# borglab/gtsfm

Measured on NVIDIA H100. Metric: image_pairs_per_sec, higher is better.
Workload: dtype f32

## Files before the change

gtsfm_b200/_lib.py:

```python
from __future__ import annotations

import ctypes as C
from pathlib import Path
from typing import Optional

import numpy as np

LIB_PATH = Path(__file__).resolve().parent / "libgtsfm_b200.so"

_lib: Optional[C.CDLL] = None


class B200Error(RuntimeError):
    pass


class LightGlueParams(C.Structure):
    _fields_ = [("depth_confidence", C.c_double), ("width_confidence", C.c_double), ("filter_threshold", C.c_double),
                ("prune_min_kpts", C.c_int), ("fp16_attention", C.c_int)]


class LightGluePair(C.Structure):
    _fields_ = [("kp0", C.c_void_p), ("desc0", C.c_void_p), ("n0", C.c_int), ("kp1", C.c_void_p), ("desc1", C.c_void_p), ("n1", C.c_int),
                ("out_matches", C.c_void_p), ("out_scores", C.c_void_p), ("out_k", C.c_int), ("out_stop_layer", C.c_int),
# ... 131 lines not shown
                ("R_error_deg", C.c_double), ("U_error_deg", C.c_double)]


class ViewGraphParams(C.Structure):
    _fields_ = [("criterion", C.c_int), ("pad_", C.c_int), ("error_threshold_deg", C.c_double)]


VG_MEDIAN, VG_MIN = 0, 1

_vp, _i, _f, _sz = C.c_void_p, C.c_int, C.c_float, C.c_size_t
_ip = C.POINTER(C.c_int)

SIGNATURES = {
    "b2_version": (_i, []),
    "b2_create": (_i, [_i, C.POINTER(_vp)]),
    "b2_destroy": (None, [_vp]),
    "b2_last_error": (C.c_char_p, [_vp]),
    "b2_launch_count": (C.c_uint64, [_vp]),
    "b2_h2d_bytes": (C.c_uint64, [_vp]),
    "b2_set_option": (C.c_int, [_vp, C.c_char_p, C.c_int64]),
    "b2_profile_start": (_i, [_vp, C.c_char_p]),
    "b2_profile_stop": (_i, [_vp, C.POINTER(C.c_double), C.POINTER(C.c_uint64), C.POINTER(C.c_double)]),
    "b2_debug_fetch": (C.c_int64, [_vp, C.c_char_p, _vp, C.c_int64]),
    "b2_debug_linear_host": (_i, [_vp, C.POINTER(LinearLaunch), C.POINTER(LinearProblem), _i]),
    "b2_debug_conv_host": (_i, [_vp, C.POINTER(ConvLayer)]),
    "b2_debug_gemm_segments_host": (_i, [_vp, _vp, _vp, _vp, _i, _i, _i, _i, _vp, _vp, _i, _vp, _vp]),
    "b2_debug_attention_host": (_i, [_vp, _i, _ip, _ip, _i, _f, _i, _vp, _vp, _vp, _vp]),
    "b2_debug_superglue_assign_host": (_i, [_vp, _i, _i, _vp, _i, _i, _f, _i, _f, _vp, _vp, _vp, _vp, _vp, _vp, _vp, _ip, _ip]),
    "b2_debug_lightglue_assign_host": (_i, [_vp, _i, _i, _vp, _i, _i, _vp, _vp, _vp, _vp, _f, _vp, _vp, _vp, _vp, _vp, _vp, _vp, _ip,
                                            _ip]),
    "b2_debug_lightglue_argmax_host": (_i, [_vp, _i, _vp, _i, _i, _vp, _vp, _vp, _vp, _vp, _ip]),
    "b2_debug_lightglue_posenc_host": (_i, [_vp, _i, _vp, _vp, _vp, _vp, _vp, _vp]),
    "b2_debug_lightglue_ln_gelu_host": (_i, [_vp, _i, _vp, _vp, _vp, _vp, _vp, _vp]),
    "b2_debug_lightglue_rowheads_host": (_i, [_vp, _i, _vp, _vp, _vp, _vp, _vp, _vp, _vp, _vp, _vp, _vp]),
    "b2_debug_lightglue_prune_host": (_i, [_vp, _i, _vp, _vp, _vp, _f, _f, _vp, _vp]),
    "b2_debug_lightglue_gather_host": (_i, [_vp, _i, _vp, _vp, _vp, _vp, _vp, _vp, _vp, _vp, _vp, _vp, _vp, _vp, _vp]),
    "b2_debug_lightglue_filter_host": (_i, [_vp, _i, _i, _vp, _vp, _vp, _f, _vp, _vp, _vp, _vp, _ip]),
    "b2_superpoint_set_weights": (_i, [_vp, _vp, _sz]),
    "b2_superpoint_detect_dev": (_i, [_vp, _vp, _i, _i, _i, _sz, _f, _i, _i, _vp, _vp, _i, _ip, C.POINTER(C.c_uint64), _vp]),
    "b2_superpoint_describe_dev": (_i, [_vp, C.c_uint64, _vp, _i, _vp, _vp]),
    "b2_superpoint_extract_dev": (_i, [_vp, _vp, _i, _i, _i, _sz, _f, _i, _i, _i, _vp, _vp, _vp, _ip, _vp]),
    "b2_superpoint_extract_async_dev": (_i, [_vp, _vp, _i, _i, _i, _sz, _f, _i, _i, _i, _vp, _vp, _vp, _vp, _vp]),
    "b2_superpoint_finish_dev": (_i, [_vp, _vp]),
    "b2_superpoint_detect_host": (_i, [_vp, _vp, _i, _i, _i, _f, _i, _i, _vp, _vp, _i, _ip, C.POINTER(C.c_uint64)]),
    "b2_superpoint_describe_host": (_i, [_vp, C.c_uint64, _vp, _i, _vp]),
    "b2_image_resize_dev": (_i, [_vp, _vp, _i, _i, _i, _sz, _vp, _i, _i, _vp]),
    "b2_lightglue_set_weights": (_i, [_vp, _vp, _sz]),
    "b2_lightglue_qkv_rows": (_i, [_vp]),
    "b2_lightglue_match_dev": (_i, [_vp, _vp, _vp, _i, _vp, _vp, _i, C.POINTER(LightGlueParams), _vp, _vp, _ip, _ip, _vp]),
    "b2_lightglue_match_host": (_i, [_vp, _vp, _vp, _i, _vp, _vp, _i, C.POINTER(LightGlueParams), _vp, _vp, _ip, _ip]),
    "b2_lightglue_match_batched_dev": (_i, [_vp, C.POINTER(LightGluePair), _i, C.POINTER(LightGlueParams), _vp]),
    "b2_lightglue_trace_count": (_i, [_vp]),
    "b2_lightglue_trace_get": (_i, [_vp, _i, _vp, _vp, _vp, _vp, _vp, _vp]),
    "b2_lightglue_encoded_bytes": (_sz, [_i]),
    "b2_lightglue_encode_batched_dev": (_i, [_vp, C.POINTER(LightGlueImage), _i, C.POINTER(LightGlueParams), _vp]),
    "b2_superglue_set_weights": (_i, [_vp, _vp, _sz]),
    "b2_superglue_match_dev": (_i, [_vp, _vp, _vp, _vp, _i, _i, _i, _vp, _vp, _vp, _i, _i, _i, _i, _f, _vp, _vp, _ip, _vp]),
    "b2_superglue_match_host": (_i, [_vp, _vp, _vp, _vp, _i, _i, _i, _vp, _vp, _vp, _i, _i, _i, _i, _f, _vp, _vp, _ip]),
    "b2_netvlad_blob_floats": (_sz, []),
    "b2_netvlad_set_weights": (_i, [_vp, _vp, _sz]),
    "b2_netvlad_describe_dev": (_i, [_vp, _vp, _i, _i, _i, _vp, _vp]),
    "b2_netvlad_describe_host": (_i, [_vp, _vp, _i, _i, _i, _vp]),
    "b2_megaloc_blob_floats": (_sz, []),
    "b2_megaloc_set_weights": (_i, [_vp, _vp, _sz]),
    "b2_megaloc_describe_dev": (_i, [_vp, _vp, _i, _i, _i, _vp, _vp]),
    "b2_megaloc_describe_host": (_i, [_vp, _vp, _i, _i, _i, _vp]),
# ... 131 lines not shown
```

gtsfm_b200/csrc/lightglue.cu:

```cuda
#include <stdlib.h>

#include "common.cuh"
#include "linear.cuh"
#include "assign_ps.cuh"

namespace {
constexpr int LG_LAYERS = 9;
constexpr size_t LG_NFLOATS = 11851601;
constexpr int D = 256;

struct SelfW {
  float *wqkv, *bqkv, *wout, *bout, *w0, *b0, *lng, *lnb, *w3, *b3;
};
struct CrossW {
  float *wqv, *bqv, *wout, *bout, *w0, *b0, *lng, *lnb, *w3, *b3;
};
struct AssignW {
  float *wm, *bm, *wf, *bf;
};
struct ConfW {
  float *w, *b;
};
}

constexpr int LG_MAX_PAIRS = 8;
constexpr int LG_MAX_SIDES = 2 * LG_MAX_PAIRS;
static_assert(LG_MAX_SIDES <= GW_MAXP && LG_MAX_SIDES <= AP_MAXP, "batch does not fit one launch");

struct LgSide {
  DevBuf x[2], xs[2], qkv, q, k, v, ctx, msg, h, hs, cs[2], sn[2], ind[2], conf, mat, src, md, rmax, rlog, ls, lsg, amax, aidx;
  int cur = 0;
  int n = 0;
  int cap = 0;
};

struct LgPair {
  bool active = false;
  int n0 = 0, n1 = 0;
  int stop = 0;
  long long* out_matches = nullptr;
  float* out_scores = nullptr;
};

struct LgTraceRec {
  int pair = 0, side = 0, layer = 0, n = 0;
  int heads = 0;
  int unconf = 0, kept = 0, stop = 0;
  std::vector<float> x, conf, mat;
  std::vector<int> ind, keep;
};

struct LightGlueState {
  bool loaded = false;
  int persist_ctas = 132;
  DevBuf wblob, wblob_h, wblob_l, errflag;
  bool use_tc = true;
  float* wr = nullptr;
  SelfW sw[LG_LAYERS];
  CrossW cw[LG_LAYERS];
  AssignW aw[LG_LAYERS];
  ConfW tw[LG_LAYERS - 1];
  float thr[LG_LAYERS];
  LgSide side[LG_MAX_SIDES];
// ... 589 lines not shown
  B2_CUDA(ctx, s->wblob.ensure(total * sizeof(float)));
  B2_CUDA(ctx, cudaMemcpy(s->wblob.p, host.data(), total * sizeof(float), cudaMemcpyHostToDevice));
  float* base = s->wblob.as<float>();
  size_t ti = 0;
  auto next = [&]() { return base + doff[ti++]; };
  s->wr = next();
  for (int i = 0; i < LG_LAYERS; ++i) {
    SelfW& a = s->sw[i];
    a.wqkv = next(), a.bqkv = next(), a.wout = next(), a.bout = next(), a.w0 = next(), a.b0 = next(), a.lng = next(),
    a.lnb = next(), a.w3 = next(), a.b3 = next();
    CrossW& c = s->cw[i];
    c.wqv = next(), c.bqv = next(), next(), next();
    c.wout = next(), c.bout = next(), c.w0 = next(), c.b0 = next(), c.lng = next(), c.lnb = next(), c.w3 = next(), c.b3 = next();
  }
  for (int i = 0; i < LG_LAYERS; ++i) {
    AssignW& a = s->aw[i];
    a.wm = next(), a.bm = next(), a.wf = next(), a.bf = next();
  }
  for (int i = 0; i < LG_LAYERS - 1; ++i) s->tw[i].w = next(), s->tw[i].b = next();
  for (int i = 0; i < LG_LAYERS; ++i) {
    double t = 0.8 + 0.1 * exp(-4.0 * i / LG_LAYERS);
    t = t < 0 ? 0 : (t > 1 ? 1 : t);
    s->thr[i] = (float)t;
  }
  B2_CUDA(ctx, s->wblob_h.ensure(total * sizeof(__half)));
  B2_CUDA(ctx, s->wblob_l.ensure(total * sizeof(__half)));
  B2_CUDA(ctx, s->errflag.ensure(16));
  B2_CUDA(ctx, cudaMemset(s->errflag.p, 0, 16));
  B2_LAUNCH(ctx, k_split_f32, (unsigned)((total + 255) / 256), 256, 0, (cudaStream_t)0, s->wblob.as<float>(), total,
            s->wblob_h.as<__half>(), s->wblob_l.as<__half>());
  B2_CHECK_LAUNCH(ctx);
  B2_CUDA(ctx, cudaDeviceSynchronize());
  B2_CUDA(ctx, cudaFuncSetAttribute(k_gemm_ws, cudaFuncAttributeMaxDynamicSharedMemorySize, (int)GW_SMEM));
  B2_CUDA(ctx, cudaFuncSetAttribute(k_flash_ps<false>, cudaFuncAttributeMaxDynamicSharedMemorySize, (int)AS_SMEM));
  B2_CUDA(ctx, cudaFuncSetAttribute(k_flash_ps<true>, cudaFuncAttributeMaxDynamicSharedMemorySize, (int)AS_SMEM));
  s->use_tc = !b2_force_simt(ctx);
  B2_CUDA(ctx, cudaFuncSetAttribute(k_flash_attn, cudaFuncAttributeMaxDynamicSharedMemorySize, (int)FA_SMEM));
  B2_CUDA(ctx, s->hread.ensure(8 * LG_MAX_PAIRS * sizeof(int)));
  B2_CUDA(ctx, s->counters.ensure(8 * LG_MAX_PAIRS * sizeof(int)));
  B2_CUDA(ctx, cudaMemset(s->counters.p, 0, 8 * LG_MAX_PAIRS * sizeof(int)));
  s->loaded = true;
  return B2_OK;
}

static inline TcWeights lg_tw(LightGlueState* s) {
  TcWeights t{s->wblob.as<float>(), s->wblob_h.as<__half>(), s->wblob_l.as<__half>(), s->errflag.as<int>(), s->use_tc};
  t.attn_part = &s->attn_part, t.attn_ml = &s->attn_ml, t.attn_cnt = &s->attn_cnt, t.sm_count = s->persist_ctas;
  return t;
}

static int lg_side_alloc(b2_context* ctx, LgSide& sd, int n, bool use_tc) {
  const size_t N = (size_t)(n > 0 ? n : 1);
  for (int i = 0; i < 2; ++i) {
    B2_CUDA(ctx, sd.x[i].ensure(N * 256 * 4));
    B2_CUDA(ctx, sd.xs[i].ensure(N * 256 * 4));
    B2_CUDA(ctx, sd.cs[i].ensure(N * 32 * 4));
    B2_CUDA(ctx, sd.sn[i].ensure(N * 32 * 4));
    B2_CUDA(ctx, sd.ind[i].ensure(N * 4));
  }
  if (!use_tc) B2_CUDA(ctx, sd.qkv.ensure(N * 768 * 4));
  B2_CUDA(ctx, sd.q.ensure(N * 256 * 4));
  B2_CUDA(ctx, sd.k.ensure(N * 256 * 4));
  B2_CUDA(ctx, sd.v.ensure(N * 256 * 4));
  B2_CUDA(ctx, sd.ctx.ensure(N * 256 * 4));
  B2_CUDA(ctx, sd.msg.ensure(N * 256 * 4));
  B2_CUDA(ctx, sd.h.ensure(N * 512 * 4));
  B2_CUDA(ctx, sd.hs.ensure(N * 512 * 4));
  B2_CUDA(ctx, sd.md.ensure(N * 256 * 4));
  DevBuf* small[] = {&sd.conf, &sd.mat, &sd.src, &sd.rmax, &sd.rlog, &sd.ls, &sd.lsg, &sd.amax, &sd.aidx};
  for (DevBuf* b : small) B2_CUDA(ctx, b->ensure(N * 4));
  sd.cur = 0;
  sd.n = n;
  sd.cap = n;
  return B2_OK;
}

struct LgActive {
  int side[LG_MAX_SIDES];
  int n = 0;
};
static LgActive lg_active_sides(const LightGlueState* s, int np) {
  LgActive a;
  for (int p = 0; p < np; ++p)
    if (s->pair[p].active) a.side[a.n++] = 2 * p, a.side[a.n++] = 2 * p + 1;
  return a;
}
static int lg_max_n(const LightGlueState* s, const LgActive& act) {
  int mx = 0;
  for (int i = 0; i < act.n; ++i) mx = s->side[act.side[i]].n > mx ? s->side[act.side[i]].n : mx;
  return mx;
}

static int lg_out_and_ffn(b2_context* ctx, cudaStream_t st, LightGlueState* s, const LgActive& act, const char* blk, const float* wout,
                          const float* bout, const float* w0, const float* b0, const float* lng, const float* lnb, const float* w3,
                          const float* b3) {
  int rc;
  const TcWeights tw = lg_tw(s);
  LinArgs o[LG_MAX_SIDES], f0[LG_MAX_SIDES], f3[LG_MAX_SIDES];
  for (int i = 0; i < act.n; ++i) {
    LgSide& sd = s->side[act.side[i]];
    const size_t e = (size_t)sd.cap * 256;
    float* x = sd.x[sd.cur].as<float>();
    LinArgs& a = o[i];
    a.a1f = sd.ctx.as<float>(), a.a1p = planes_of(sd.ctx, e), a.lda1 = 256, a.K1 = 256, a.w = wout, a.ldb = 256, a.bias = bout;
    a.cf = sd.msg.as<float>(), a.ldc = 256, a.cp = planes_of(sd.msg, e), a.ldch = 256, a.M = sd.n, a.N = 256;
    LinArgs& f = f0[i];
    f.a1f = x, f.a1p = planes_of(sd.xs[sd.cur], e), f.lda1 = 256, f.K1 = 256;
    f.a2f = sd.msg.as<float>(), f.a2p = planes_of(sd.msg, e), f.lda2 = 256, f.K2 = 256;
    f.w = w0, f.ldb = 512, f.bias = b0, f.cf = sd.h.as<float>(), f.ldc = 512, f.tc_want_f32 = true, f.M = sd.n, f.N = 512;
    LinArgs& c = f3[i];
    c.a1f = sd.h.as<float>(), c.a1p = planes_of(sd.hs, (size_t)sd.cap * 512), c.lda1 = 512, c.K1 = 512, c.w = w3, c.ldb = 512, c.bias = b3;
    c.resid = x, c.ldr = 256;
    c.cf = x, c.ldc = 256, c.tc_want_f32 = true, c.cp = planes_of(sd.xs[sd.cur], e), c.ldch = 256, c.M = sd.n, c.N = 256;
  }
  const std::string site(blk);
  if ((rc = run_linear(ctx, st, tw, o, act.n, (site + "_out").c_str()))) return rc;
  if ((rc = run_linear(ctx, st, tw, f0, act.n, (site + "_ffn0").c_str()))) return rc;
  {
    JobList<LnJob> lj{};
    for (int i = 0; i < act.n; ++i) {
      LgSide& sd = s->side[act.side[i]];
      const Pl hs = planes_of(sd.hs, (size_t)sd.cap * 512);
      lj.j[i] = {sd.h.as<float>(), sd.n, s->use_tc ? hs.hi : (__half*)nullptr, s->use_tc ? hs.lo : (__half*)nullptr};
    }
    const int mx = lg_max_n(s, act);
    if (mx > 0) {
      B2_LAUNCH(ctx, k_lg_ln_gelu, dim3(cdiv(mx, 8), act.n), 256, 0, st, lj, lng, lnb);
      B2_CHECK_LAUNCH(ctx);
    }
  }
  return run_linear(ctx, st, tw, f3, act.n, (site + "_ffn3").c_str());
}

static int lg_self_layer(b2_context* ctx, cudaStream_t st, LightGlueState* s, const LgActive& act, int layer, bool fp16_attn) {
  const SelfW& w = s->sw[layer];
  const TcWeights tw = lg_tw(s);
  int rc;
  LinArgs q[LG_MAX_SIDES];
  for (int i = 0; i < act.n; ++i) {
    LgSide& sd = s->side[act.side[i]];
    const size_t e = (size_t)sd.cap * 256;
    LinArgs& a = q[i];
    a.a1f = sd.x[sd.cur].as<float>(), a.a1p = planes_of(sd.xs[sd.cur], e), a.lda1 = 256, a.K1 = 256;
    a.w = w.wqkv, a.ldb = 256, a.bias = w.bqkv, a.M = sd.n, a.N = 768;
    if (s->use_tc) {
      a.seg_n = 256, a.seg_p[0] = planes_of(sd.q, e), a.seg_p[1] = planes_of(sd.k, e), a.seg_p[2] = planes_of(sd.v, e);
      a.rot_mask = 3, a.cs = sd.cs[sd.cur].as<float>(), a.sn = sd.sn[sd.cur].as<float>();
      a.head_major = 1, a.lo_unscaled = 1;
    } else {
      a.cf = sd.qkv.as<float>(), a.ldc = 768;
    }
  }
  if ((rc = run_linear(ctx, st, tw, q, act.n, "lg_self_qkv"))) return rc;
  const int mx = lg_max_n(s, act);
  if (!s->use_tc && mx > 0) {
    JobList<RotJob> rj{};
// ... 593 lines not shown
    const int pb = cdiv(mx * 32, 1024);
    B2_LAUNCH(ctx, k_lg_posenc, dim3(pb < 16 ? pb : 16, np), 1024, 0, d.st, pj, dwr);
    B2_CHECK_LAUNCH(ctx);
  }
  return d.finish("b2_debug_lightglue_posenc_host");
}

extern "C" int b2_debug_lightglue_ln_gelu_host(b2_context* ctx, int np, const int* n, const float* g, const float* b, float* h,
                                               uint16_t* hi, uint16_t* lo) {
  int mx, rc;
  if (!ctx || !g || !b || !h || !hi != !lo || lg_dbg_sizes(n, np, &mx)) return B2_ERR_ARG;
  std::lock_guard<std::mutex> lk(ctx->mu);
  cudaSetDevice(ctx->device);
  LgDbg d{ctx, ctx->stream};
  JobList<LnJob> lj{};
  float *dg, *db;
  if ((rc = d.put(g, 512, false, &dg)) || (rc = d.put(b, 512, false, &db))) return rc;
  for (int i = 0, o = 0; i < np; o += n[i++]) {
    LnJob& j = lj.j[i];
    const size_t e = 512 * (size_t)o, ne = 512 * (size_t)n[i];
    j.n = n[i];
    uint16_t *dh = nullptr, *dl = nullptr;
    if ((rc = d.put(h + e, ne, true, &j.h)) || (hi && ((rc = d.put(hi + e, ne, true, &dh)) || (rc = d.put(lo + e, ne, true, &dl)))))
      return rc;
    j.hi = reinterpret_cast<__half*>(dh), j.lo = reinterpret_cast<__half*>(dl);
  }
  if (mx > 0) {
    B2_LAUNCH(ctx, k_lg_ln_gelu, dim3(cdiv(mx, 8), np), 256, 0, d.st, lj, dg, db);
    B2_CHECK_LAUNCH(ctx);
  }
  return d.finish("b2_debug_lightglue_ln_gelu_host");
}

extern "C" int b2_debug_lightglue_rowheads_host(b2_context* ctx, int np, const int* n, const int* mode, const float* x, const float* w1,
                                                const float* b1, const float* w2, const float* b2, float* o1, float* o2, float* zraw) {
  int mx, rc;
  if (!ctx || !mode || !x || !o1 || !o2 || !zraw || !w1 != !b1 || !w2 != !b2 || lg_dbg_sizes(n, np, &mx)) return B2_ERR_ARG;
  std::lock_guard<std::mutex> lk(ctx->mu);
  cudaSetDevice(ctx->device);
  LgDbg d{ctx, ctx->stream};
  JobList<HeadJob> hj{};
  float *dw1, *db1, *dw2, *db2;
  if ((rc = d.put(w1, 256, false, &dw1)) || (rc = d.put(b1, 1, false, &db1)) || (rc = d.put(w2, 256, false, &dw2)) ||
      (rc = d.put(b2, 1, false, &db2)))
    return rc;
  for (int i = 0, o = 0; i < np; o += n[i++]) {
    HeadJob& j = hj.j[i];
    float *dx, *d1, *d2, *dz;
    if ((rc = d.put(x + 256 * (size_t)o, 256 * (size_t)n[i], false, &dx)) || (rc = d.put(o1 + o, (size_t)n[i], true, &d1)) ||
        (rc = d.put(o2 + o, (size_t)n[i], true, &d2)) || (rc = d.put(zraw + o, (size_t)n[i], true, &dz)))
      return rc;
    const bool h2 = (mode[i] & 1) && dw2;
    j = {dx, n[i], h2 ? dw2 : nullptr, h2 ? db2 : nullptr, d1, (mode[i] & 2) ? d2 : nullptr, (mode[i] & 4) ? dz : nullptr};
  }
  if (mx > 0) {
    B2_LAUNCH(ctx, k_lg_rowheads, dim3(cdiv(mx, 8), np), 256, 0, d.st, hj, dw1, db1);
    B2_CHECK_LAUNCH(ctx);
  }
  return d.finish("b2_debug_lightglue_rowheads_host");
}

extern "C" int b2_debug_lightglue_prune_host(b2_context* ctx, int np, const int* n, const float* conf, const float* mat, float thr,
                                             float keep_thr, int* src, int* counters) {
  int mx, rc;
  if (!ctx || !conf || !mat || !src || !counters || lg_dbg_sizes(n, np, &mx)) return B2_ERR_ARG;
  std::lock_guard<std::mutex> lk(ctx->mu);
// ... 108 lines not shown
```

gtsfm_b200/csrc/linear.cuh:

```cuda
#pragma once
#include "attn_ps.cuh"
#include "common.cuh"
#include "gemm.cuh"
#include "gemm_ws.cuh"

struct TcWeights {
  const float* f;
  const __half* h;
  const __half* l;
  int* err;
  bool use_tc;
  DevBuf* attn_part = nullptr;
  DevBuf* attn_ml = nullptr;
  DevBuf* attn_cnt = nullptr;
  int sm_count = 132;
};

struct Pl {
  __half* hi;
  __half* lo;
};
static inline Pl planes_of(const DevBuf& b, size_t elems) { return {b.as<__half>(), b.as<__half>() + elems}; }

struct LinArgs {
  const float* a1f = nullptr;
  Pl a1p{nullptr, nullptr};
  int lda1 = 0, K1 = 0;
  const float* a2f = nullptr;
  Pl a2p{nullptr, nullptr};
  int lda2 = 0, K2 = 0;
  const float* w = nullptr;
  const float* bf = nullptr;
  Pl bp{nullptr, nullptr};
  int ldb = 0;
  const float* bias = nullptr;
  float scale = 1.f;
  const float* resid = nullptr;
  int ldr = 0;
  float* cf = nullptr;
  int ldc = 0;
  Pl cp{nullptr, nullptr};
  int ldch = 0;
  int head_major = 0;
  bool tc_want_f32 = false;
  int relu = 0;
  int gelu = 0;
  int lo_unscaled = 0;
  int M = 0, N = 0;
  int seg_n = 0;
  float* seg_f[GW_SEGS] = {};
  Pl seg_p[GW_SEGS] = {};
  int rot_mask = 0;
  const float *cs = nullptr, *sn = nullptr;
};

static int run_linear(b2_context* ctx, cudaStream_t st, const TcWeights& tw, const LinArgs* a, int np, const char* site = nullptr) {
  if (np <= 0) return B2_OK;
  if (np > GW_MAXP) return b2_fail(ctx, B2_ERR_ARG, "run_linear: too many problems in one launch");
  const LinArgs& a0 = a[0];
  const int nseg = a0.seg_n > 0 ? a0.N / a0.seg_n : 1;
  if (a0.seg_n > 0 && (a0.seg_n % GW_N || a0.N != nseg * a0.seg_n || nseg > GW_SEGS || !a0.head_major || a0.resid || a0.tc_want_f32 ||
                       (a0.rot_mask && (!a0.cs || !a0.sn))))
    return b2_fail(ctx, B2_ERR_ARG, "run_linear: column segments need N = seg_n x (<= 3), seg_n % 128 == 0, head-major planes, "
                                    "no residual or fp32 output, and a rotary table when rotary is on");
  if (!tw.use_tc) {
    if (a0.rot_mask) return b2_fail(ctx, B2_ERR_ARG, "run_linear: the rotary epilogue exists on the wgmma path only");
    for (int i = 0; i < np; ++i) {
      const LinArgs& x = a[i];
      if (x.M <= 0 || x.N <= 0) continue;
      if (x.gelu) return b2_fail(ctx, B2_ERR_ARG, "run_linear: the GELU epilogue exists on the wgmma path only");
      if (x.K1 % GB_K || x.K2 % GB_K || x.lda1 % 4 || x.lda2 % 4 || x.ldb % 4)
        return b2_fail(ctx, B2_ERR_ARG, "run_linear: the SIMT GEMM needs K1, K2 multiples of 16 and lda1, lda2, ldb multiples of 4");
    }
    for (int i = 0; i < np; ++i) {
      const LinArgs& x = a[i];
      if (x.M <= 0 || x.N <= 0) continue;
      for (int s = 0; s < nseg; ++s) {
        const int c0 = s * x.seg_n;
        GemmArgs g{};
        g.A1 = x.a1f, g.lda1 = x.lda1, g.K1 = x.K1, g.A2 = x.a2f, g.lda2 = x.lda2, g.K2 = x.K2;
        g.B = (x.w ? x.w : x.bf) + (size_t)c0 * x.ldb, g.ldb = x.ldb, g.C = x.seg_n ? x.seg_f[s] : x.cf, g.ldc = x.ldc, g.M = x.M;
        g.N = x.seg_n ? x.seg_n : x.N;
        g.bias = x.bias ? x.bias + c0 : nullptr, g.resid = x.resid, g.ldr = x.ldr, g.scale = x.scale, g.head_major = x.head_major;
        g.relu = x.relu;
        int rc = launch_gemm(ctx, st, g);
        if (rc) return rc;
      }
    }
    return B2_OK;
  }
  if (a0.K1 % GW_K || a0.K2 % GW_K) return b2_fail(ctx, B2_ERR_ARG, "run_linear: the wgmma GEMM needs K1 and K2 multiples of 64");
  if (!tma_encoder()) return b2_fail(ctx, B2_ERR_CUDA, "cuTensorMapEncodeTiled is not available (driver too old?)");
  const bool per_b = a0.w == nullptr;
  static thread_local GemmWsMaps maps;
  GemmWsArgs q{};
  double work = 0.0;
  bool ok = true;
  int nz = 0, tiles = 0;
  for (int i = 0; i < np; ++i) {
    const LinArgs& x = a[i];
    if (x.M <= 0 || x.N <= 0) continue;
    ok = ok && tma_map_2d(&maps.a1h[nz], x.a1p.hi, x.M, x.K1, x.lda1, GW_M) && tma_map_2d(&maps.a1l[nz], x.a1p.lo, x.M, x.K1, x.lda1, GW_M);
    if (x.K2 > 0)
      ok = ok && tma_map_2d(&maps.a2h[nz], x.a2p.hi, x.M, x.K2, x.lda2, GW_M) && tma_map_2d(&maps.a2l[nz], x.a2p.lo, x.M, x.K2, x.lda2, GW_M);
    if (per_b || nz == 0) {
      const __half *bh, *bl;
      if (x.w) {
        const size_t off = (size_t)(x.w - tw.f);
        bh = tw.h + off, bl = tw.l + off;
      } else {
        bh = x.bp.hi, bl = x.bp.lo;
      }
      ok = ok && tma_map_2d(&maps.bh[nz], bh, x.N, x.K1 + x.K2, x.ldb, GW_N) && tma_map_2d(&maps.bl[nz], bl, x.N, x.K1 + x.K2, x.ldb, GW_N);
    }
    GemmProblem& pr = q.p[nz];
    pr.resid = x.resid, pr.C = x.tc_want_f32 ? x.cf : nullptr, pr.M = x.M, pr.N = x.N, pr.ldc = x.ldc;
    for (int s = 0; s < GW_SEGS; ++s) {
      const Pl p = x.seg_n ? (s < nseg ? x.seg_p[s] : Pl{nullptr, nullptr}) : (s == 0 ? x.cp : Pl{nullptr, nullptr});
      pr.Ch[s] = p.hi, pr.Cl[s] = p.lo;
    }
    pr.cs = x.cs, pr.sn = x.sn;
    {
      auto al16 = [](const void* q) { return (reinterpret_cast<uintptr_t>(q) & 15) == 0; };
// ... 112 lines not shown
```

include/gtsfm_b200.h:

```cpp
#ifndef GTSFM_B200_H
#define GTSFM_B200_H

#include <stddef.h>
#include <stdint.h>

#ifdef __cplusplus
extern "C" {
#endif

typedef struct b2_context b2_context;

int b2_version(void);
int b2_create(int device, b2_context** out);
void b2_destroy(b2_context* ctx);
const char* b2_last_error(const b2_context* ctx);
uint64_t b2_launch_count(const b2_context* ctx);
uint64_t b2_h2d_bytes(const b2_context* ctx);
int b2_set_option(b2_context* ctx, const char* name, int64_t value);
int b2_profile_start(b2_context* ctx, const char* kernel_prefix);
int b2_profile_stop(b2_context* ctx, double* total_ms, uint64_t* launches, double* work);
int64_t b2_debug_fetch(b2_context* ctx, const char* name, float* host_out, int64_t max_floats);

typedef struct b2_linear_problem {
  const float* a1; int lda1;
// ... 12 lines not shown
  int relu, gelu, head_major, lo_unscaled;
  int resid_in_place;
} b2_linear_launch;
int b2_debug_linear_host(b2_context* ctx, const b2_linear_launch* launch, const b2_linear_problem* problems, int np);
typedef struct b2_conv_layer {
  int path;
  int dilation, pool, relu, ctas;
  int height, width, cin, cout;
  const float* in;
  const float* weight;
  const float* bias;
  float* out;
  uint16_t* out_hi; uint16_t* out_lo;
} b2_conv_layer;
int b2_debug_conv_host(b2_context* ctx, const b2_conv_layer* layer);
int b2_debug_gemm_segments_host(b2_context* ctx, const float* A, const float* B, const float* bias, int M, int K, int nseg,
                                int rot_mask, const float* cs, const float* sn, int separate, uint16_t* out_hi,
                                uint16_t* out_lo);
int b2_debug_attention_host(b2_context* ctx, int np, const int* nq, const int* nk, int heads, float scale, int single,
                            const float* q, const float* k, const float* v, float* o);
int b2_debug_superglue_assign_host(b2_context* ctx, int path, int ctas, const float* Z, int M, int N, float alpha, int iters,
                                   float threshold, float* u, float* v, float* best0, int* arg0, int* arg1, uint32_t* out_matches,
                                   float* out_scores, int* out_k, int* out_path);
int b2_debug_lightglue_assign_host(b2_context* ctx, int path, int ctas, const float* sim, int M, int N, const float* z0,
                                   const float* z1, const int* ind0, const int* ind1, float threshold, float* row_stats,
                                   float* col_stats, float* best0, int* arg0, int* arg1, int64_t* out_matches, float* out_scores,
                                   int* out_k, int* out_path);
int b2_debug_lightglue_argmax_host(b2_context* ctx, int path, const float* sim, int M, int N, const float* z0, const float* z1,
                                   float* best0, int* arg0, int* arg1, int* out_path);
int b2_debug_lightglue_posenc_host(b2_context* ctx, int np, const int* n, const float* kp, const float* wr, float* cs, float* sn,
                                   int* ind);
int b2_debug_lightglue_ln_gelu_host(b2_context* ctx, int np, const int* n, const float* g, const float* b, float* h, uint16_t* hi,
                                    uint16_t* lo);
int b2_debug_lightglue_rowheads_host(b2_context* ctx, int np, const int* n, const int* mode, const float* x, const float* w1,
                                     const float* b1, const float* w2, const float* b2, float* o1, float* o2, float* zraw);
int b2_debug_lightglue_prune_host(b2_context* ctx, int np, const int* n, const float* conf, const float* mat, float thr,
                                  float keep_thr, int* src, int* counters);
int b2_debug_lightglue_gather_host(b2_context* ctx, int np, const int* n, const int* cnt, const int* src, const float* x,
                                   const float* cs, const float* sn, const int* ind, const uint16_t* planes, float* x2, float* cs2,
                                   float* sn2, int* ind2, uint16_t* planes2);
int b2_debug_lightglue_filter_host(b2_context* ctx, int m, int n, const float* best0, const int* a0, const int* a1, float th,
                                   const int* ind0, const int* ind1, int64_t* out_matches, float* out_scores, int* out_k);

int b2_superpoint_set_weights(b2_context* ctx, const float* host_blob, size_t n_floats);

int b2_superpoint_detect_dev(b2_context* ctx, const uint8_t* image, int height, int width, int channels, size_t pitch,
                             float keypoint_threshold, int nms_radius, int border, float* out_xy, float* out_score,
                             int cap, int* out_n, uint64_t* out_map_token, void* stream);
int b2_superpoint_describe_dev(b2_context* ctx, uint64_t map_token, const float* xy, int n, float* out_desc, void* stream);
int b2_superpoint_extract_dev(b2_context* ctx, const uint8_t* image, int height, int width, int channels, size_t pitch,
                              float keypoint_threshold, int nms_radius, int border, int max_keypoints, float* out_xy,
                              float* out_score, float* out_desc, int* out_n, void* stream);
int b2_superpoint_extract_async_dev(b2_context* ctx, const uint8_t* image, int height, int width, int channels, size_t pitch,
                                    float threshold, int nms_radius, int border, int max_keypoints, float* out_xy,
                                    float* out_score, float* out_desc, int* out_n_pinned, void* stream);
int b2_superpoint_finish_dev(b2_context* ctx, void* stream);

int b2_superpoint_detect_host(b2_context* ctx, const uint8_t* image, int height, int width, int channels,
                              float keypoint_threshold, int nms_radius, int border, float* out_xy, float* out_score,
                              int cap, int* out_n, uint64_t* out_map_token);
int b2_superpoint_describe_host(b2_context* ctx, uint64_t map_token, const float* xy, int n, float* out_desc);

int b2_image_resize_dev(b2_context* ctx, const uint8_t* src, int height, int width, int channels, size_t pitch, uint8_t* dst,
                        int new_height, int new_width, void* stream);

int b2_lightglue_set_weights(b2_context* ctx, const float* host_blob, size_t n_floats);
// ... 344 lines not shown
```

Before: 129.7.

## Fuse LayerNorm+GELU prologue into warp-specialized FFN output GEMM

Adds a warp-specialized wgmma kernel that computes LayerNorm and GELU on the 512-wide FFN hidden rows inside the GEMM prologue. It writes the split fp16 hi/lo A operand straight into swizzled shared memory instead of running a separate ln_gelu kernel that stores the hs planes to global memory. This removes one launch and a round trip of the hidden activations through global memory per block, and drops the hs buffer. In exchange, each tile re-reads H twice (once for row statistics, once for normalization), and producer, MMA and epilogue warps now depend on a more complex mbarrier handshake.

```diff
diff --git a/gtsfm_b200/_lib.py b/gtsfm_b200/_lib.py
--- a/gtsfm_b200/_lib.py
+++ b/gtsfm_b200/_lib.py
@@ -187,6 +187,7 @@
     "b2_debug_lightglue_argmax_host": (_i, [_vp, _i, _vp, _i, _i, _vp, _vp, _vp, _vp, _vp, _ip]),
     "b2_debug_lightglue_posenc_host": (_i, [_vp, _i, _vp, _vp, _vp, _vp, _vp, _vp]),
     "b2_debug_lightglue_ln_gelu_host": (_i, [_vp, _i, _vp, _vp, _vp, _vp, _vp, _vp]),
+    "b2_debug_lightglue_ffn3_host": (_i, [_vp, _i, _vp, _i, _vp, _vp, _vp, _vp, _vp, _vp, _vp, _vp]),
     "b2_debug_lightglue_rowheads_host": (_i, [_vp, _i, _vp, _vp, _vp, _vp, _vp, _vp, _vp, _vp, _vp, _vp]),
     "b2_debug_lightglue_prune_host": (_i, [_vp, _i, _vp, _vp, _vp, _f, _f, _vp, _vp]),
     "b2_debug_lightglue_gather_host": (_i, [_vp, _i, _vp, _vp, _vp, _vp, _vp, _vp, _vp, _vp, _vp, _vp, _vp, _vp, _vp]),
diff --git a/gtsfm_b200/csrc/gemm_ws_ln.cuh b/gtsfm_b200/csrc/gemm_ws_ln.cuh
--- /dev/null
+++ b/gtsfm_b200/csrc/gemm_ws_ln.cuh
@@ -0,0 +1,270 @@
+#pragma once
+#include "gemm_ws.cuh"
+
+constexpr int GL_M = 64, GL_K = 512, GL_N = 256;
+constexpr int GL_A_BYTES = GL_M * GL_K * 2;
+constexpr int GL_CHUNK_BYTES = GL_M * GW_K * 2;
+constexpr int GL_B_BYTES = GW_N * GW_K * 2;
+constexpr int GL_STAGE_BYTES = 2 * GL_B_BYTES;
+constexpr int GL_STAGES = 2;
+constexpr int GL_NK = GL_K / GW_K;
+constexpr int GL_PITCH = GW_N + 4;
+constexpr int GL_STG_BYTES = GL_M * GL_PITCH * 4;
+constexpr int GL_THREADS = 512;
+constexpr size_t GL_SMEM = 2 * GL_A_BYTES + GL_STAGES * GL_STAGE_BYTES + GL_STG_BYTES + 1024  + 256  +
+                         GL_M * 8 ;
+static_assert(GL_SMEM <= 232448, "k_gemm_ws_ln does not fit the 227 KB of shared memory a CTA may have");
+
+struct GemmLnProblem {
+  const float* H;
+  const float* resid;
+  float* C;
+  __half *Ch, *Cl;
+  int M;
+  int tile_end;
+};
+struct GemmLnMaps {
+  CUtensorMap bh, bl;
+};
+struct GemmLnArgs {
+  GemmLnProblem p[GW_MAXP];
+  int nprob, tiles;
+  const float *bias, *gamma, *beta;
+  float scale;
+  int* err_flag;
+};
+
+static __global__ void __launch_bounds__(GL_THREADS, 1) k_gemm_ws_ln(const __grid_constant__ GemmLnMaps maps, const __grid_constant__ GemmLnArgs g) {
+  extern __shared__ unsigned char gl_raw[];
+  const uint32_t raw = tc::smem_u32(gl_raw);
+  const uint32_t smem0 = (raw + 1023u) & ~1023u;
+  unsigned char* sm = gl_raw + (smem0 - raw);
+  const uint32_t sA = smem0;
+  const uint32_t sB = smem0 + 2 * GL_A_BYTES;
+  float* stg = reinterpret_cast<float*>(sm + 2 * GL_A_BYTES + GL_STAGES * GL_STAGE_BYTES);
+  uint64_t* full = reinterpret_cast<uint64_t*>(sm + 2 * GL_A_BYTES + GL_STAGES * GL_STAGE_BYTES + GL_STG_BYTES);
+  uint64_t* empty = full + GL_STAGES;
+  uint64_t* sfull = empty + GL_STAGES;
+  uint64_t* sempty = sfull + 1;
+  uint64_t* afull = sempty + 1;
+  uint64_t* aempty = afull + GL_NK;
+  float2* stats = reinterpret_cast<float2*>(sm + 2 * GL_A_BYTES + GL_STAGES * GL_STAGE_BYTES + GL_STG_BYTES + 256);
+
+  const int t = threadIdx.x, warp = t >> 5, lane = t & 31;
+  if (t == 0) {
+    for (int s = 0; s < GL_STAGES; ++s) tc::mbar_init(&full[s], 1), tc::mbar_init(&empty[s], 4);
+    tc::mbar_init(sfull, 128);
+    tc::mbar_init(sempty, 128);
+    for (int k = 0; k < GL_NK; ++k) tc::mbar_init(&afull[k], 128), tc::mbar_init(&aempty[k], 4);
+    tc::fence_mbar_init();
+    tc::tma_prefetch_desc(&maps.bh);
+    tc::tma_prefetch_desc(&maps.bl);
+  }
+  __syncthreads();
+  bool ok = true;
+
+  auto decode = [&](int tile, int& z, int& m0) {
+    z = 0;
+    while (z + 1 < g.nprob && tile >= g.p[z].tile_end) ++z;
+    m0 = (tile - (z ? g.p[z - 1].tile_end : 0)) * GL_M;
+  };
+
+  if (warp >= 12) {
+    asm volatile("setmaxnreg.dec.sync.aligned.u32 40;\n" ::: "memory");
+    if (warp == 12 && lane == 0) {
+      int gk = 0;
+      for (int tile = blockIdx.x; tile < g.tiles; tile += gridDim.x)
+        for (int h = 0; h < 2; ++h)
+          for (int kc = 0; kc < GL_NK; ++kc, ++gk) {
+            const int s = gk % GL_STAGES;
+            if (gk >= GL_STAGES) ok = tc::mbar_wait(&empty[s], ((gk / GL_STAGES) - 1) & 1) && ok;
+            const uint32_t dst = sB + s * GL_STAGE_BYTES;
+            tc::mbar_expect_tx(&full[s], GL_STAGE_BYTES);
+            tc::tma_load_2d(dst, &maps.bh, &full[s], kc * GW_K, h * GW_N);
+            tc::tma_load_2d(dst + GL_B_BYTES, &maps.bl, &full[s], kc * GW_K, h * GW_N);
+          }
+    }
+  } else if (warp < 4) {
+    asm volatile("setmaxnreg.inc.sync.aligned.u32 184;\n" ::: "memory");
+    const int r0 = warp * 16 + (lane >> 2);
+    const int c2 = (lane & 3) * 2;
+    int gk = 0, it = 0, ht = 0;
+    for (int tile = blockIdx.x; tile < g.tiles; tile += gridDim.x, ++it) {
+#pragma unroll 1
+      for (int h = 0; h < 2; ++h, ++ht) {
+        float acc0[64], acc1[64];
+        for (int kc = 0; kc < GL_NK; ++kc, ++gk) {
+          const int s = gk % GL_STAGES;
+          if (h == 0) ok = tc::mbar_wait(&afull[kc], it & 1) && ok;
+          ok = tc::mbar_wait(&full[s], (gk / GL_STAGES) & 1) && ok;
+          const uint32_t aH = sA + kc * GL_CHUNK_BYTES, aL = aH + GL_A_BYTES;
+          const uint32_t bH = sB + s * GL_STAGE_BYTES, bL = bH + GL_B_BYTES;
+          const uint64_t dAh = tc::wg_desc_sw128(aH), dAl = tc::wg_desc_sw128(aL), dBh = tc::wg_desc_sw128(bH), dBl = tc::wg_desc_sw128(bL);
+          tc::wg_fence();
+#pragma unroll
+          for (int ks = 0; ks < GW_K / 16; ++ks) {
+            const uint64_t adv = (uint64_t)(ks * 2);
+            const uint32_t first = (kc == 0 && ks == 0) ? 0u : 1u;
+            tc::wg_ss_n128(acc0, dAh + adv, dBh + adv, first);
+            tc::wg_ss_n128(acc1, dAh + adv, dBl + adv, first);
+            tc::wg_ss_n128(acc1, dAl + adv, dBh + adv, 1u);
+          }
+          tc::wg_commit();
+          if (kc > 0) {
+            tc::wg_wait<1>();
+            if (lane == 0) {
+              tc::mbar_arrive(&empty[(gk - 1) % GL_STAGES]);
+              if (h == 1) tc::mbar_arrive(&aempty[kc - 1]);
+            }
+          }
+        }
+        tc::wg_wait<0>();
+        if (lane == 0) {
+          tc::mbar_arrive(&empty[(gk - 1) % GL_STAGES]);
+          if (h == 1) tc::mbar_arrive(&aempty[GL_NK - 1]);
+        }
+        if (ht > 0) ok = tc::mbar_wait(sempty, (ht - 1) & 1) && ok;
+#pragma unroll
+        for (int j = 0; j < 16; ++j)
+#pragma unroll
+          for (int hh = 0; hh < 2; ++hh) {
+            const int i = 4 * j + 2 * hh;
+            *reinterpret_cast<float2*>(stg + (r0 + 8 * hh) * GL_PITCH + 8 * j + c2) =
+                make_float2(fmaf(acc1[i], tc::LO_INV, acc0[i]), fmaf(acc1[i + 1], tc::LO_INV, acc0[i + 1]));
+          }
+        tc::mbar_arrive(sfull);
+      }
+    }
+  } else if (warp < 8) {
+    asm volatile("setmaxnreg.inc.sync.aligned.u32 168;\n" ::: "memory");
+    const int lw = warp - 4, lt = t - 128;
+    const float* __restrict__ gam = g.gamma;
+    const float* __restrict__ bet = g.beta;
+    int it = 0;
+    for (int tile = blockIdx.x; tile < g.tiles; tile += gridDim.x, ++it) {
+      int z, m0;
+      decode(tile, z, m0);
+      const float* H = g.p[z].H;
+      const int rows = min(GL_M, g.p[z].M - m0);
+      auto load = [&](int r, float4* v) {
+        if (r < rows) {
+          const float4* row = reinterpret_cast<const float4*>(H + (size_t)(m0 + r) * GL_K);
+#pragma unroll
+          for (int i = 0; i < 4; ++i) v[i] = row[lane + 32 * i];
+        } else {
+#pragma unroll
+          for (int i = 0; i < 4; ++i) v[i] = make_float4(0.f, 0.f, 0.f, 0.f);
+        }
+      };
+      auto row_stats = [&](int r, const float4* v) {
+        float s = 0.f;
+#pragma unroll
+        for (int i = 0; i < 4; ++i) s += v[i].x + v[i].y + v[i].z + v[i].w;
+        float mean = warp_sum(s) / 512.0f;
+        float q = 0.f;
+#pragma unroll
+        for (int i = 0; i < 4; ++i) {
+          float a = v[i].x - mean, bq = v[i].y - mean, c = v[i].z - mean, d = v[i].w - mean;
+          q += a * a + bq * bq + c * c + d * d;
+        }
+        float rstd = 1.0f / sqrtf(warp_sum(q) / 512.0f + 1e-5f);
+        if (lane == 0) stats[r] = make_float2(mean, rstd);
+      };
+#pragma unroll 1
+      for (int r = lw; r < GL_M; r += 8) {
+        float4 va[4], vb[4];
+        load(r, va);
+        load(r + 4, vb);
+        row_stats(r, va);
+        row_stats(r + 4, vb);
+      }
+      asm volatile("bar.sync 1, 128;" ::: "memory");
+      const int cq = lt & 15, rq = lt >> 4;
+#pragma unroll 1
+      for (int kc = 0; kc < GL_NK; ++kc) {
+        const int c0 = kc * GW_K + 4 * cq;
+        float4 v[GL_M / 8];
+#pragma unroll
+        for (int k = 0; k < GL_M / 8; ++k) {
+          const int r = rq + 8 * k;
+          v[k] = r < rows ? *reinterpret_cast<const float4*>(H + (size_t)(m0 + r) * GL_K + c0) : make_float4(0.f, 0.f, 0.f, 0.f);
+        }
+        const float4 gg = *reinterpret_cast<const float4*>(gam + c0), bb = *reinterpret_cast<const float4*>(bet + c0);
+        if (it > 0) ok = tc::mbar_wait(&aempty[kc], (it - 1) & 1) && ok;
+#pragma unroll
+        for (int k = 0; k < GL_M / 8; ++k) {
+          const int r = rq + 8 * k;
+          const float2 st = stats[r];
+          const float mean = st.x, rstd = st.y;
+          float e[4] = {(v[k].x - mean) * rstd * gg.x + bb.x, (v[k].y - mean) * rstd * gg.y + bb.y,
+                        (v[k].z - mean) * rstd * gg.z + bb.z, (v[k].w - mean) * rstd * gg.w + bb.w};
+#pragma unroll
+          for (int j = 0; j < 4; ++j) e[j] = 0.5f * e[j] * (1.0f + erff(e[j] * 0.70710678118654752440f));
+          uint32_t h01, l01, h23, l23;
+          tc::split2(e[0], e[1], h01, l01);
+          tc::split2(e[2], e[3], h23, l23);
+          const uint32_t off = kc * GL_CHUNK_BYTES + r * 128 + ((((cq >> 1) ^ (r & 7)) << 4) | ((cq & 1) * 8));
+          asm volatile("st.shared.v2.u32 [%0], {%1, %2};" ::"r"(sA + off), "r"(h01), "r"(h23) : "memory");
+          asm volatile("st.shared.v2.u32 [%0], {%1, %2};" ::"r"(sA + GL_A_BYTES + off), "r"(l01), "r"(l23) : "memory");
+        }
+        tc::fence_proxy_async();
+        tc::mbar_arrive(&afull[kc]);
+      }
+      asm volatile("bar.sync 1, 128;" ::: "memory");
+    }
+  } else {
+    asm volatile("setmaxnreg.dec.sync.aligned.u32 120;\n" ::: "memory");
+    const int ew = warp - 8;
+    const float scale = g.scale;
+    int ht = 0;
+    for (int tile = blockIdx.x; tile < g.tiles; tile += gridDim.x) {
+      int z, m0;
+      decode(tile, z, m0);
+      const GemmLnProblem& pb = g.p[z];
+      const float* resid = pb.resid;
+      float* C = pb.C;
+      __half *Ch = pb.Ch, *Cl = pb.Cl;
+      const int rows = min(GL_M, pb.M - m0);
+#pragma unroll 1
+      for (int h = 0; h < 2; ++h, ++ht) {
+        const int n = h * GW_N + 4 * lane;
+        float b4[4] = {0.f, 0.f, 0.f, 0.f};
+        if (g.bias)
+#pragma unroll
+          for (int e = 0; e < 4; ++e) b4[e] = __ldg(g.bias + n + e);
+        float4 rr[GW_RB];
+        auto load_rows = [&](int rb) {
+#pragma unroll
+          for (int i = 0; i < GW_RB; ++i)
+            if (rb + GW_EW * i < rows) rr[i] = *reinterpret_cast<const float4*>(resid + (size_t)(m0 + rb + GW_EW * i) * GL_N + n);
+        };
+        if (resid) load_rows(ew);
+        ok = tc::mbar_wait(sfull, ht & 1) && ok;
+        for (int rb = ew; rb < rows; rb += GW_EW * GW_RB) {
+          if (resid && rb != ew) load_rows(rb);
+#pragma unroll
+          for (int i = 0; i < GW_RB; ++i) {
+            const int r = rb + GW_EW * i;
+            if (r >= rows) break;
+            const float4 a = *reinterpret_cast<const float4*>(stg + r * GL_PITCH + 4 * lane);
+            float v[4] = {a.x, a.y, a.z, a.w};
+#pragma unroll
+            for (int e = 0; e < 4; ++e) v[e] = (v[e] + b4[e]) * scale;
+            if (resid) v[0] += rr[i].x, v[1] += rr[i].y, v[2] += rr[i].z, v[3] += rr[i].w;
+            const size_t off = (size_t)(m0 + r) * GL_N + n;
+            if (C) *reinterpret_cast<float4*>(C + off) = make_float4(v[0], v[1], v[2], v[3]);
+            if (Ch) {
+              uint32_t h01, l01, h23, l23;
+              tc::split2(v[0], v[1], h01, l01);
+              tc::split2(v[2], v[3], h23, l23);
+              *reinterpret_cast<uint2*>(Ch + off) = make_uint2(h01, h23);
+              *reinterpret_cast<uint2*>(Cl + off) = make_uint2(l01, l23);
+            }
+          }
+        }
+        tc::mbar_arrive(sempty);
+      }
+    }
+  }
+  if (!ok && g.err_flag) *g.err_flag = 1;
+}
diff --git a/gtsfm_b200/csrc/lightglue.cu b/gtsfm_b200/csrc/lightglue.cu
--- a/gtsfm_b200/csrc/lightglue.cu
+++ b/gtsfm_b200/csrc/lightglue.cu
@@ -28,7 +28,7 @@
 static_assert(LG_MAX_SIDES <= GW_MAXP && LG_MAX_SIDES <= AP_MAXP, "batch does not fit one launch");
 
 struct LgSide {
-  DevBuf x[2], xs[2], qkv, q, k, v, ctx, msg, h, hs, cs[2], sn[2], ind[2], conf, mat, src, md, rmax, rlog, ls, lsg, amax, aidx;
+  DevBuf x[2], xs[2], qkv, q, k, v, ctx, msg, h, cs[2], sn[2], ind[2], conf, mat, src, md, rmax, rlog, ls, lsg, amax, aidx;
   int cur = 0;
   int n = 0;
   int cap = 0;
@@ -684,6 +684,7 @@
   B2_CHECK_LAUNCH(ctx);
   B2_CUDA(ctx, cudaDeviceSynchronize());
   B2_CUDA(ctx, cudaFuncSetAttribute(k_gemm_ws, cudaFuncAttributeMaxDynamicSharedMemorySize, (int)GW_SMEM));
+  B2_CUDA(ctx, cudaFuncSetAttribute(k_gemm_ws_ln, cudaFuncAttributeMaxDynamicSharedMemorySize, (int)GL_SMEM));
   B2_CUDA(ctx, cudaFuncSetAttribute(k_flash_ps<false>, cudaFuncAttributeMaxDynamicSharedMemorySize, (int)AS_SMEM));
   B2_CUDA(ctx, cudaFuncSetAttribute(k_flash_ps<true>, cudaFuncAttributeMaxDynamicSharedMemorySize, (int)AS_SMEM));
   s->use_tc = !b2_force_simt(ctx);
@@ -717,7 +718,6 @@
   B2_CUDA(ctx, sd.ctx.ensure(N * 256 * 4));
   B2_CUDA(ctx, sd.msg.ensure(N * 256 * 4));
   B2_CUDA(ctx, sd.h.ensure(N * 512 * 4));
-  B2_CUDA(ctx, sd.hs.ensure(N * 512 * 4));
   B2_CUDA(ctx, sd.md.ensure(N * 256 * 4));
   DevBuf* small[] = {&sd.conf, &sd.mat, &sd.src, &sd.rmax, &sd.rlog, &sd.ls, &sd.lsg, &sd.amax, &sd.aidx};
   for (DevBuf* b : small) B2_CUDA(ctx, b->ensure(N * 4));
@@ -761,19 +761,19 @@
     f.a2f = sd.msg.as<float>(), f.a2p = planes_of(sd.msg, e), f.lda2 = 256, f.K2 = 256;
     f.w = w0, f.ldb = 512, f.bias = b0, f.cf = sd.h.as<float>(), f.ldc = 512, f.tc_want_f32 = true, f.M = sd.n, f.N = 512;
     LinArgs& c = f3[i];
-    c.a1f = sd.h.as<float>(), c.a1p = planes_of(sd.hs, (size_t)sd.cap * 512), c.lda1 = 512, c.K1 = 512, c.w = w3, c.ldb = 512, c.bias = b3;
+    c.a1f = sd.h.as<float>(), c.lda1 = 512, c.K1 = 512, c.w = w3, c.ldb = 512, c.bias = b3;
+    if (s->use_tc) c.ln_g = lng, c.ln_b = lnb;
     c.resid = x, c.ldr = 256;
     c.cf = x, c.ldc = 256, c.tc_want_f32 = true, c.cp = planes_of(sd.xs[sd.cur], e), c.ldch = 256, c.M = sd.n, c.N = 256;
   }
   const std::string site(blk);
   if ((rc = run_linear(ctx, st, tw, o, act.n, (site + "_out").c_str()))) return rc;
   if ((rc = run_linear(ctx, st, tw, f0, act.n, (site + "_ffn0").c_str()))) return rc;
-  {
+  if (!s->use_tc) {
     JobList<LnJob> lj{};
     for (int i = 0; i < act.n; ++i) {
       LgSide& sd = s->side[act.side[i]];
-      const Pl hs = planes_of(sd.hs, (size_t)sd.cap * 512);
-      lj.j[i] = {sd.h.as<float>(), sd.n, s->use_tc ? hs.hi : (__half*)nullptr, s->use_tc ? hs.lo : (__half*)nullptr};
+      lj.j[i] = {sd.h.as<float>(), sd.n, nullptr, nullptr};
     }
     const int mx = lg_max_n(s, act);
     if (mx > 0) {
@@ -1433,6 +1433,66 @@
   return d.finish("b2_debug_lightglue_ln_gelu_host");
 }
 
+extern "C" int b2_debug_lightglue_ffn3_host(b2_context* ctx, int np, const int* n, int fused, const float* h, const float* w3, const float* b3,
+                                            const float* g, const float* b, float* x, uint16_t* xs_hi, uint16_t* xs_lo) {
+  int mx, rc;
+  if (!ctx || !h || !w3 || !b3 || !g || !b || !x || !xs_hi || !xs_lo || (fused != 0 && fused != 1) || lg_dbg_sizes(n, np, &mx))
+    return B2_ERR_ARG;
+  std::lock_guard<std::mutex> lk(ctx->mu);
+  cudaSetDevice(ctx->device);
+  LgDbg d{ctx, ctx->stream};
+  float *dw, *db3, *dg, *db;
+  if ((rc = d.put(w3, 256 * 512, false, &dw)) || (rc = d.put(b3, 256, false, &db3)) || (rc = d.put(g, 512, false, &dg)) ||
+      (rc = d.put(b, 512, false, &db)))
+    return rc;
+  size_t tot = 0;
+  for (int i = 0; i < np; ++i) tot += (size_t)n[i];
+  DevBuf wh, wl, err, hs;
+  B2_CUDA(ctx, wh.ensure(256 * 512 * 2));
+  B2_CUDA(ctx, wl.ensure(256 * 512 * 2));
+  B2_CUDA(ctx, err.ensure(16));
+  B2_CUDA(ctx, cudaMemsetAsync(err.p, 0, 16, d.st));
+  B2_CUDA(ctx, hs.ensure((tot > 0 ? tot : 1) * 512 * 2 * 2));
+  B2_LAUNCH(ctx, k_split_f32, 256 * 512 / 256, 256, 0, d.st, dw, (size_t)256 * 512, wh.as<__half>(), wl.as<__half>());
+  B2_CHECK_LAUNCH(ctx);
+  JobList<LnJob> lj{};
+  LinArgs la[LG_MAX_SIDES];
+  for (int i = 0, o = 0; i < np; o += n[i++]) {
+    float *dh, *dx;
+    uint16_t *dxh, *dxl;
+    const size_t e = 256 * (size_t)o, ne = 256 * (size_t)n[i];
+    if ((rc = d.put(h + 2 * e, 2 * ne, false, &dh)) || (rc = d.put(x + e, ne, true, &dx)) || (rc = d.put(xs_hi + e, ne, true, &dxh)) ||
+        (rc = d.put(xs_lo + e, ne, true, &dxl)))
+      return rc;
+    LinArgs& c = la[i];
+    c.a1f = dh, c.lda1 = 512, c.K1 = 512, c.w = dw, c.ldb = 512, c.bias = db3;
+    c.resid = dx, c.ldr = 256, c.cf = dx, c.ldc = 256, c.tc_want_f32 = true, c.M = n[i], c.N = 256;
+    c.cp = {reinterpret_cast<__half*>(dxh), reinterpret_cast<__half*>(dxl)}, c.ldch = 256;
+    if (fused) {
+      c.ln_g = dg, c.ln_b = db;
+    } else {
+      __half* hi = hs.as<__half>() + 2 * e;
+      c.a1p = {hi, hi + tot * 512};
+      lj.j[i] = {dh, n[i], c.a1p.hi, c.a1p.lo};
+    }
+  }
+  if (!fused && mx > 0) {
+    B2_LAUNCH(ctx, k_lg_ln_gelu, dim3(cdiv(mx, 8), np), 256, 0, d.st, lj, dg, db);
+    B2_CHECK_LAUNCH(ctx);
+  }
+  B2_CUDA(ctx, cudaFuncSetAttribute(k_gemm_ws, cudaFuncAttributeMaxDynamicSharedMemorySize, (int)GW_SMEM));
+  B2_CUDA(ctx, cudaFuncSetAttribute(k_gemm_ws_ln, cudaFuncAttributeMaxDynamicSharedMemorySize, (int)GL_SMEM));
+  TcWeights tw{dw, wh.as<__half>(), wl.as<__half>(), err.as<int>(), true};
+  tw.sm_count = ctx->sm_count;
+  if ((rc = run_linear(ctx, d.st, tw, la, np))) return rc;
+  if ((rc = d.finish("b2_debug_lightglue_ffn3_host"))) return rc;
+  int e = 0;
+  B2_CUDA(ctx, cudaMemcpyAsync(&e, err.p, 4, cudaMemcpyDeviceToHost, d.st));
+  B2_CUDA(ctx, cudaStreamSynchronize(d.st));
+  if (e) return b2_fail(ctx, B2_ERR_STATE, "wgmma pipeline timed out on an mbarrier (kernel bug)");
+  return B2_OK;
+}
+
 extern "C" int b2_debug_lightglue_rowheads_host(b2_context* ctx, int np, const int* n, const int* mode, const float* x, const float* w1,
                                                 const float* b1, const float* w2, const float* b2, float* o1, float* o2, float* zraw) {
   int mx, rc;
diff --git a/gtsfm_b200/csrc/linear.cuh b/gtsfm_b200/csrc/linear.cuh
--- a/gtsfm_b200/csrc/linear.cuh
+++ b/gtsfm_b200/csrc/linear.cuh
@@ -3,6 +3,7 @@
 #include "common.cuh"
 #include "gemm.cuh"
 #include "gemm_ws.cuh"
+#include "gemm_ws_ln.cuh"
 
 struct TcWeights {
   const float* f;
@@ -52,7 +53,49 @@
   Pl seg_p[GW_SEGS] = {};
   int rot_mask = 0;
   const float *cs = nullptr, *sn = nullptr;
-};
+  const float *ln_g = nullptr, *ln_b = nullptr;
+};
+
+static int run_linear_ln(b2_context* ctx, cudaStream_t st, const TcWeights& tw, const LinArgs* a, int np, const char* site) {
+  const LinArgs& a0 = a[0];
+  if (!a0.ln_b || a0.K1 != GL_K || a0.K2 || !a0.w || a0.seg_n || a0.head_major || a0.relu || a0.gelu || a0.lo_unscaled || a0.rot_mask)
+    return b2_fail(ctx, B2_ERR_ARG, "run_linear: the LayerNorm operand needs gamma and beta, K1 = 512 and no second K segment, a weight "
+                                    "B operand, and a plain row-major epilogue");
+  if (!tma_encoder()) return b2_fail(ctx, B2_ERR_CUDA, "cuTensorMapEncodeTiled is not available (driver too old?)");
+  auto al16 = [](const void* q) { return (reinterpret_cast<uintptr_t>(q) & 15) == 0; };
+  auto al8 = [](const void* q) { return (reinterpret_cast<uintptr_t>(q) & 7) == 0; };
+  GemmLnMaps maps;
+  {
+    const size_t off = (size_t)(a0.w - tw.f);
+    if (!tma_map_2d(&maps.bh, tw.h + off, GL_N, GL_K, a0.ldb, GW_N) || !tma_map_2d(&maps.bl, tw.l + off, GL_N, GL_K, a0.ldb, GW_N))
+      return b2_fail(ctx, B2_ERR_CUDA, "cuTensorMapEncodeTiled failed");
+  }
+  GemmLnArgs q{};
+  double work = 0.0;
+  int nz = 0, tiles = 0;
+  for (int i = 0; i < np; ++i) {
+    const LinArgs& x = a[i];
+    if (x.M <= 0 || x.N <= 0) continue;
+    const float* C = x.tc_want_f32 ? x.cf : nullptr;
+    if (x.N != GL_N || !x.a1f || x.lda1 != GL_K || !al16(x.a1f) || (x.resid && (x.ldr != GL_N || !al16(x.resid))) ||
+        (C && (x.ldc != GL_N || !al16(C))) || (x.cp.hi && (x.ldch != GL_N || !al8(x.cp.hi) || !al8(x.cp.lo))) || (!C && !x.cp.hi))
+      return b2_fail(ctx, B2_ERR_ARG, "run_linear: the LayerNorm operand needs N = 256, a 16-byte aligned fp32 A of pitch 512, and "
+                                      "aligned outputs and residual of pitch 256");
+    GemmLnProblem& pr = q.p[nz];
+    pr.H = x.a1f, pr.resid = x.resid, pr.C = const_cast<float*>(C), pr.Ch = x.cp.hi, pr.Cl = x.cp.lo, pr.M = x.M;
+    tiles += cdiv(x.M, GL_M);
+    pr.tile_end = tiles;
+    work += 2.0 * x.M * GL_N * GL_K;
+    ++nz;
+  }
+  if (nz == 0) return B2_OK;
+  q.nprob = nz, q.tiles = tiles, q.bias = a0.bias, q.gamma = a0.ln_g, q.beta = a0.ln_b, q.scale = a0.scale, q.err_flag = tw.err;
+  const std::string name = site ? std::string("k_gemm_ws/") + site : std::string("k_gemm_ws");
+  b2_prof_work(ctx, name.c_str(), work);
+  B2_LAUNCH_NAMED(ctx, name.c_str(), k_gemm_ws_ln, tiles < tw.sm_count ? tiles : tw.sm_count, GL_THREADS, GL_SMEM, st, maps, q);
+  B2_CHECK_LAUNCH(ctx);
+  return B2_OK;
+}
 
 static int run_linear(b2_context* ctx, cudaStream_t st, const TcWeights& tw, const LinArgs* a, int np, const char* site = nullptr) {
   if (np <= 0) return B2_OK;
@@ -65,6 +108,7 @@
                                     "no residual or fp32 output, and a rotary table when rotary is on");
   if (!tw.use_tc) {
     if (a0.rot_mask) return b2_fail(ctx, B2_ERR_ARG, "run_linear: the rotary epilogue exists on the wgmma path only");
+    if (a0.ln_g) return b2_fail(ctx, B2_ERR_ARG, "run_linear: the LayerNorm operand exists on the wgmma path only");
     for (int i = 0; i < np; ++i) {
       const LinArgs& x = a[i];
       if (x.M <= 0 || x.N <= 0) continue;
@@ -89,6 +133,7 @@
     }
     return B2_OK;
   }
+  if (a0.ln_g || a0.ln_b) return run_linear_ln(ctx, st, tw, a, np, site);
   if (a0.K1 % GW_K || a0.K2 % GW_K) return b2_fail(ctx, B2_ERR_ARG, "run_linear: the wgmma GEMM needs K1 and K2 multiples of 64");
   if (!tma_encoder()) return b2_fail(ctx, B2_ERR_CUDA, "cuTensorMapEncodeTiled is not available (driver too old?)");
   const bool per_b = a0.w == nullptr;
diff --git a/include/gtsfm_b200.h b/include/gtsfm_b200.h
--- a/include/gtsfm_b200.h
+++ b/include/gtsfm_b200.h
@@ -68,6 +68,8 @@
                                    int* ind);
 int b2_debug_lightglue_ln_gelu_host(b2_context* ctx, int np, const int* n, const float* g, const float* b, float* h, uint16_t* hi,
                                     uint16_t* lo);
+int b2_debug_lightglue_ffn3_host(b2_context* ctx, int np, const int* n, int fused, const float* h, const float* w3, const float* b3,
+                                 const float* g, const float* b, float* x, uint16_t* xs_hi, uint16_t* xs_lo);
 int b2_debug_lightglue_rowheads_host(b2_context* ctx, int np, const int* n, const int* mode, const float* x, const float* w1,
                                      const float* b1, const float* w2, const float* b2, float* o1, float* o2, float* zraw);
 int b2_debug_lightglue_prune_host(b2_context* ctx, int np, const int* n, const float* conf, const float* mat, float thr,
```

Result: no change. 129.0 (median of 6 runs) (-0.6%).
